# sigp/consensus-specs

Measured on AMD Instinct MI355X. Metric: BLS sig verifications/sec (whole node), higher is better.
Workload: dtype u32 (381-bit Montgomery, 14x28-bit limbs in u32 words); 1 GPU; C2: 65536 independent bls_verify deposit PoP checks per GPU (domain=3, 1/16 tampered); global_batch=65536, parallelism=dp1 (independent items, no collective), batches_in_flight=1, subgroup_policy=pyecc

## Files before the change

consensus-specs_amd/csrc/bls381_field.hpp:

```cpp
#pragma once
#include "bls381_defs.hpp"
#include "bls381_consts.hpp"

namespace bls381 {

#if defined(BLS_COUNT_OPS) && !defined(__HIP_DEVICE_COMPILE__)
inline thread_local uint64_t g_fp_macs = 0;
#define BLS_COUNT_MACS(k) (g_fp_macs += (k))
#else
#define BLS_COUNT_MACS(k) ((void)0)
#endif
#if !defined(__HIP_DEVICE_COMPILE__) && !defined(__HIP__)
inline uint64_t g_inv_fallbacks = 0;
#define BLS_COUNT_INV_FALLBACK() (++g_inv_fallbacks)
#else
#define BLS_COUNT_INV_FALLBACK() ((void)0)
#endif

BLS_INLINE fp_t fp_zero() { fp_t r; for (int i = 0; i < 14; ++i) r.w[i] = 0; return r; }
BLS_INLINE fp_t fp_one() { return FP_ONE_M; }

BLS_INLINE void fp_carry(int32_t (&t)[14]) {
#pragma unroll
  for (int i = 0; i < 13; ++i) {
    t[i + 1] += t[i] >> 28;
    t[i] &= (int32_t)FP_MASK;
  }
}

template <int KMAX>
BLS_INLINE fp_t fp_reduce_lc(const uint32_t (&s)[14]) {
  static_assert(KMAX >= 1 && KMAX <= 8, "value bound");
  int32_t t[14];
  if (KMAX <= 2) {
    const uint32_t m = (int32_t)s[13] > (int32_t)Q2_LIMBS[13] ? ~0u : 0u;
#pragma unroll
    for (int i = 0; i < 14; ++i) t[i] = (int32_t)(s[i] - (Q2_LIMBS[i] & m));
  } else {
    const int32_t top = (int32_t)s[13] > 0 ? (int32_t)s[13] : 0;
    const uint32_t k = (uint32_t)(((uint64_t)(uint32_t)top * LC_DIV_MAGIC) >> 40);
#pragma unroll
    for (int i = 0; i < 14; ++i) t[i] = (int32_t)(s[i] + k * NQ2_LIMBS[i]);
  }
  fp_carry(t);
  if (BLS_ANY(t[13] >= (int32_t)Q2_LIMBS[13])) {
    int32_t e[14];
#pragma unroll
    for (int i = 0; i < 14; ++i) e[i] = t[i] - (int32_t)Q2_LIMBS[i];
    fp_carry(e);
    const bool ge = e[13] >= 0;
#pragma unroll
    for (int i = 0; i < 14; ++i) t[i] = ge ? e[i] : t[i];
  }
  fp_t r;
#pragma unroll
  for (int i = 0; i < 14; ++i) r.w[i] = (uint32_t)t[i];
  return r;
}

BLS_INLINE fp_t fp_add(const fp_t& a, const fp_t& b) {
  uint32_t s[14];
#pragma unroll
  for (int i = 0; i < 14; ++i) s[i] = a.w[i] + b.w[i];
  return fp_reduce_lc<2>(s);
}

BLS_INLINE fp_t fp_sub(const fp_t& a, const fp_t& b) {
  uint32_t s[14];
#pragma unroll
  for (int i = 0; i < 14; ++i) s[i] = a.w[i] + Q2B_LIMBS[i] - b.w[i];
  return fp_reduce_lc<2>(s);
}

BLS_INLINE fp_t fp_neg(const fp_t& a) {
  uint32_t s[14];
#pragma unroll
  for (int i = 0; i < 14; ++i) s[i] = Q2B_LIMBS[i] - a.w[i];
  return fp_reduce_lc<2>(s);
}

BLS_INLINE fp_t fp_dbl(const fp_t& a) {
  uint32_t s[14];
#pragma unroll
  for (int i = 0; i < 14; ++i) s[i] = a.w[i] << 1;
  return fp_reduce_lc<2>(s);
}

BLS_INLINE fp_t fp_add_sub(const fp_t& a, const fp_t& b, const fp_t& c) {
  uint32_t s[14];
#pragma unroll
  for (int i = 0; i < 14; ++i) s[i] = a.w[i] + b.w[i] + Q2B_LIMBS[i] - c.w[i];
  return fp_reduce_lc<3>(s);
}

BLS_INLINE fp_t fp_add3(const fp_t& a, const fp_t& b, const fp_t& c) {
  uint32_t s[14];
#pragma unroll
  for (int i = 0; i < 14; ++i) s[i] = a.w[i] + b.w[i] + c.w[i];
  return fp_reduce_lc<3>(s);
}

BLS_INLINE fp_t fp_sub2(const fp_t& a, const fp_t& b, const fp_t& c) {
  uint32_t s[14];
#pragma unroll
  for (int i = 0; i < 14; ++i) s[i] = a.w[i] + Q4B_LIMBS[i] - b.w[i] - c.w[i];
  return fp_reduce_lc<3>(s);
}

BLS_INLINE fp_t fp_3m2(const fp_t& X, const fp_t& x) {
  uint32_t s[14];
#pragma unroll
  for (int i = 0; i < 14; ++i) s[i] = 3u * X.w[i] + Q4B_LIMBS[i] - (x.w[i] << 1);
  return fp_reduce_lc<5>(s);
}
BLS_INLINE fp_t fp_3p2(const fp_t& X, const fp_t& x) {
  uint32_t s[14];
#pragma unroll
  for (int i = 0; i < 14; ++i) s[i] = 3u * X.w[i] + (x.w[i] << 1);
  return fp_reduce_lc<5>(s);
}
BLS_INLINE fp_t fp_3pm2(const fp_t& X, const fp_t& x, bool minus) {
  uint32_t s[14];
#pragma unroll
  for (int i = 0; i < 14; ++i) {
    const uint32_t x2 = x.w[i] << 1;
    s[i] = 3u * X.w[i] + (minus ? Q4B_LIMBS[i] - x2 : x2);
  }
  return fp_reduce_lc<5>(s);
}

template <int NS> BLS_INLINE uint32_t lc_offset(int i) {
  static_assert(NS >= 2 && NS <= 4, "offsets for two to four subtracted values");
  return NS == 2 ? Q4B_LIMBS[i] : NS == 3 ? Q8T_LIMBS[i] : Q10F_LIMBS[i];
}
constexpr int lc_kmax(int na, int ns) { return na + (ns <= 2 ? ns : ns + 1); }

template <int NA, int NS>
BLS_INLINE fp_t fp_lc(const fp_t* const (&add)[NA], const fp_t* const (&sub)[NS]) {
  static_assert(NA + NS <= 7 && lc_kmax(NA, NS) <= 8, "fp_reduce_lc's limb and value bounds");
  uint32_t s[14];
#pragma unroll
  for (int i = 0; i < 14; ++i) {
    uint32_t v = lc_offset<NS>(i);
#pragma unroll
    for (int j = 0; j < NA; ++j) v += add[j]->w[i];
#pragma unroll
    for (int j = 0; j < NS; ++j) v -= sub[j]->w[i];
    s[i] = v;
  }
  return fp_reduce_lc<lc_kmax(NA, NS)>(s);
}

BLS_INLINE fp_t fp_add_lazy(const fp_t& a, const fp_t& b) {
  fp_t r;
#pragma unroll
  for (int i = 0; i < 14; ++i) r.w[i] = a.w[i] + b.w[i];
  return r;
}

BLS_INLINE fp_t fp_reduce_once(const fp_t& s) {
  int32_t b[14];
#pragma unroll
  for (int i = 0; i < 14; ++i) b[i] = (int32_t)s.w[i] - (int32_t)Q_LIMBS[i];
  fp_carry(b);
  const bool neg = b[13] < 0;
  fp_t r;
#pragma unroll
  for (int i = 0; i < 14; ++i) r.w[i] = neg ? s.w[i] : (uint32_t)b[i];
  return r;
}

BLS_INLINE bool fp_is_zero(const fp_t& a) {
  uint32_t z = 0, e = 0;
#pragma unroll
  for (int i = 0; i < 14; ++i) { z |= a.w[i]; e |= a.w[i] ^ Q_LIMBS[i]; }
  return z == 0 || e == 0;
}

BLS_INLINE bool fp_eq(const fp_t& a, const fp_t& b) { return fp_is_zero(fp_sub(a, b)); }

BLS_INLINE fp_t fp_half(const fp_t& a) {
  const uint32_t odd = a.w[0] & 1u;
  int32_t s[14];
#pragma unroll
  for (int i = 0; i < 14; ++i) s[i] = (int32_t)(a.w[i] + (odd ? Q_LIMBS[i] : 0u));
  fp_carry(s);
  fp_t r;
#pragma unroll
  for (int i = 0; i < 13; ++i) r.w[i] = ((uint32_t)s[i] >> 1) | (((uint32_t)s[i + 1] & 1u) << 27);
  r.w[13] = (uint32_t)s[13] >> 1;
  return r;
}

BLS_INLINE uint64_t fp_mac(uint64_t acc, uint32_t x, uint32_t y) { return BLS_KEEP_ORDER(acc + (uint64_t)x * y); }

template <class F>
BLS_INLINE fp_t fp_mont_columns(const F& col) {
  uint32_t m[14];
  fp_t r;
  uint64_t c = 0;
#pragma unroll
  for (int k = 0; k < 27; ++k) {
    uint64_t acc = col(k, c);
#pragma unroll
    for (int i = (k > 13 ? k - 13 : 0); i < k && i < 14; ++i) acc = fp_mac(acc, m[i], Q_LIMBS[k - i]);
    if (k < 14) {
      m[k] = ((uint32_t)acc * Q_INV28) & FP_MASK;
      acc = fp_mac(acc, m[k], Q_LIMBS[0]);
    } else {
      r.w[k - 14] = (uint32_t)acc & FP_MASK;
    }
    c = acc >> 28;
  }
  r.w[13] = (uint32_t)c & FP_MASK;
  return r;
}

BLS_INLINE fp_t fp_mul_body(const fp_t& a, const fp_t& b) {
  return fp_mont_columns([&](int k, uint64_t acc) {
#pragma unroll
    for (int i = (k > 13 ? k - 13 : 0); i <= k && i < 14; ++i) acc = fp_mac(acc, a.w[i], b.w[k - i]);
    return acc;
  });
}

BLS_INLINE fp_t fp_sqr_body(const fp_t& a) {
  uint32_t a2[14];
#pragma unroll
  for (int i = 0; i < 14; ++i) a2[i] = a.w[i] << 1;
  return fp_mont_columns([&](int k, uint64_t acc) {
#pragma unroll
    for (int i = (k > 13 ? k - 13 : 0); 2 * i < k; ++i) acc = fp_mac(acc, a2[i], a.w[k - i]);
    if ((k & 1) == 0) acc = fp_mac(acc, a.w[k / 2], a.w[k / 2]);
    return acc;
  });
}

#if defined(__clang__)
typedef uint32_t fpv_t __attribute__((ext_vector_type(14)));
BLS_INLINE fpv_t fp_pack(const fp_t& a) {
  fpv_t v;
#pragma unroll
  for (int k = 0; k < 14; ++k) v[k] = a.w[k];
  return v;
}
BLS_INLINE fp_t fp_unpack(const fpv_t& v) {
  fp_t a;
#pragma unroll
  for (int k = 0; k < 14; ++k) a.w[k] = v[k];
  return a;
}
BLS_NOINLINE fpv_t fp_mul_call(fpv_t a, fpv_t b) { return fp_pack(fp_mul_body(fp_unpack(a), fp_unpack(b))); }
BLS_NOINLINE fpv_t fp_sqr_call(fpv_t a) { return fp_pack(fp_sqr_body(fp_unpack(a))); }
BLS_INLINE fp_t fp_mul(const fp_t& a, const fp_t& b) { return fp_unpack(fp_mul_call(fp_pack(a), fp_pack(b))); }
BLS_INLINE fp_t fp_sqr(const fp_t& a) { return fp_unpack(fp_sqr_call(fp_pack(a))); }
#else
BLS_NOINLINE fp_t fp_mul(fp_t a, fp_t b) { BLS_COUNT_MACS(392); return fp_mul_body(a, b); }
BLS_NOINLINE fp_t fp_sqr(fp_t a) { BLS_COUNT_MACS(301); return fp_sqr_body(a); }
#endif

BLS_INLINE fp_t fp_mul_small(const fp_t& a, int k) {
  if (k <= 8) {
    uint32_t s[14];
#pragma unroll
    for (int i = 0; i < 14; ++i) s[i] = (uint32_t)k * a.w[i];
    return fp_reduce_lc<8>(s);
  }
  fp_t r = a;
  fp_t acc = fp_zero();
  bool first = true;
  while (k) {
    if (k & 1) { acc = first ? r : fp_add(acc, r); first = false; }
    k >>= 1;
    if (k) r = fp_dbl(r);
  }
  return acc;
}

BLS_DEV_INLINE fp_t fp_pow_limbs(const fp_t& a, const uint32_t* e, int nbits) {
  fp_t r = FP_ONE_M;
  for (int i = nbits - 1; i >= 0; --i) {
    r = fp_sqr(r);
    if ((e[i >> 5] >> (i & 31)) & 1u) r = fp_mul(r, a);
  }
  return r;
}

BLS_HD inline fp_t fp_pow_qm3d4(const fp_t a) {
  const fp_t a2 = fp_sqr(a);
  const fp_t t1 = a, t3 = fp_mul(t1, a2), t5 = fp_mul(t3, a2), t7 = fp_mul(t5, a2);
  const fp_t t9 = fp_mul(t7, a2), t11 = fp_mul(t9, a2), t13 = fp_mul(t11, a2), t15 = fp_mul(t13, a2);
  fp_t r = FP_ONE_M;
  for (int k = 0; k < POW_QM3D4_NSTEPS; ++k) {
    for (int j = POW_QM3D4_SQR[k]; j > 0; --j) r = fp_sqr(r);
    switch (POW_QM3D4_DIG[k]) {
      case 1: r = fp_mul(r, t1); break;
      case 3: r = fp_mul(r, t3); break;
      case 5: r = fp_mul(r, t5); break;
      case 7: r = fp_mul(r, t7); break;
      case 9: r = fp_mul(r, t9); break;
      case 11: r = fp_mul(r, t11); break;
      case 13: r = fp_mul(r, t13); break;
      case 15: r = fp_mul(r, t15); break;
      default: break;
    }
  }
  return r;
}

BLS_HD inline fp_t fp_inv(const fp_t am);

BLS_DEV_INLINE bool fp_sqrt(fp_t& r, const fp_t& a) {
  r = fp_mul(fp_pow_qm3d4(a), a);
  return fp_eq(fp_sqr(r), a);
}

BLS_INLINE fp_t fp_to_mont(const fp_t& plain) { return fp_mul(plain, FP_R2); }
BLS_INLINE fp_t fp_from_mont(const fp_t& m) {
  fp_t one = fp_zero();
  one.w[0] = 1;
  return fp_reduce_once(fp_mul(m, one));
}

BLS_INLINE bool fp_plain_lt_q(const fp_t& a) {
  int32_t b[14];
#pragma unroll
  for (int i = 0; i < 14; ++i) b[i] = (int32_t)a.w[i] - (int32_t)Q_LIMBS[i];
  fp_carry(b);
  return b[13] < 0;
}

BLS_INLINE bool fp_plain_is_zero(const fp_t& a) {
  uint32_t z = 0;
#pragma unroll
  for (int i = 0; i < 14; ++i) z |= a.w[i];
  return z == 0;
}

BLS_INLINE bool fp_plain_gt(const fp_t& a, const fp_t& b) {
  int32_t d[14];
#pragma unroll
  for (int i = 0; i < 14; ++i) d[i] = (int32_t)b.w[i] - (int32_t)a.w[i];
  fp_carry(d);
// ... 748 lines not shown
```

consensus-specs_amd/csrc/bls381_lazy.hpp:

```cpp
#pragma once
#include "bls381_field.hpp"

namespace bls381 {

struct wide_t { int64_t c[28]; };
typedef int32_t lv_t[14];

constexpr int WIDE_OFF_SHIFT = 22;

BLS_INLINE void wz_init(wide_t& T) {
#pragma unroll
  for (int k = 0; k < 28; ++k) T.c[k] = 0;
#pragma unroll
  for (int j = 0; j < 14; ++j) T.c[13 + j] = (int64_t)Q_LIMBS[j] << WIDE_OFF_SHIFT;
}

BLS_INLINE void wmac(wide_t& T, const lv_t& x, const lv_t& y) {
  BLS_COUNT_MACS(196);
#pragma unroll
  for (int i = 0; i < 14; ++i)
#pragma unroll
    for (int j = 0; j < 14; ++j) T.c[i + j] += (int64_t)x[i] * (int64_t)y[j];
}

BLS_INLINE void wmac_init(wide_t& T, const lv_t& x, const lv_t& y) {
  BLS_COUNT_MACS(196);
#pragma unroll
  for (int i = 0; i < 14; ++i)
#pragma unroll
    for (int j = 0; j < 14; ++j) {
      const int k = i + j;
      const int64_t p = (int64_t)x[i] * (int64_t)y[j];
      if (i == 0 || j == 13)
        T.c[k] = p + ((k >= 13) ? ((int64_t)Q_LIMBS[k - 13] << WIDE_OFF_SHIFT) : 0);
      else
        T.c[k] += p;
    }
  T.c[27] = 0;
}

BLS_INLINE void wsqr_k(wide_t& T, const lv_t& x, int32_t k) {
  BLS_COUNT_MACS(105);
#pragma unroll
  for (int i = 0; i < 14; ++i) {
    const int32_t d = k * x[i], c = 2 * k * x[i];
    T.c[2 * i] += (int64_t)d * (int64_t)x[i];
#pragma unroll
    for (int j = i + 1; j < 14; ++j) T.c[i + j] += (int64_t)c * (int64_t)x[j];
  }
}

BLS_INLINE fp_t wredc(wide_t& T) {
  BLS_COUNT_MACS(196);
#pragma unroll
  for (int i = 0; i < 14; ++i) {
    const uint32_t m = ((uint32_t)T.c[i] * Q_INV28) & FP_MASK;
#pragma unroll
    for (int j = 0; j < 14; ++j) T.c[i + j] = (int64_t)((uint64_t)T.c[i + j] + (uint64_t)m * Q_LIMBS[j]);
    T.c[i + 1] += T.c[i] >> 28;
  }
  fp_t r;
  int64_t c = 0;
#pragma unroll
  for (int j = 0; j < 14; ++j) {
    const int64_t v = T.c[14 + j] + c;
    r.w[j] = (uint32_t)v & FP_MASK;
    c = v >> 28;
  }
  return r;
}

BLS_INLINE void lv_from(lv_t& r, const fp_t& a) {
#pragma unroll
  for (int k = 0; k < 14; ++k) r[k] = (int32_t)a.w[k];
}

BLS_INLINE fp_t fp_6p2(const fp_t& X, const fp_t& x) {
  uint32_t s[14];
#pragma unroll
  for (int i = 0; i < 14; ++i) s[i] = 6u * X.w[i] + (x.w[i] << 1);
  return fp_reduce_lc<6>(s);
}

BLS_INLINE fp_t fp_6p2_3m2(bool six, const fp_t& P, const fp_t& S, const fp_t& x) {
  uint32_t s[14];
#pragma unroll
  for (int i = 0; i < 14; ++i) {
    const uint32_t x2 = x.w[i] << 1;
    s[i] = six ? 6u * P.w[i] + x2 : 3u * S.w[i] + Q4B_LIMBS[i] - x2;
  }
  return fp_reduce_lc<6>(s);
}


BLS_INLINE fp_t lz_xi_mul(bool p, const fp_t& a0, const fp_t& a1, const fp_t& b0, const fp_t& b1) {
  lv_t x1, y1, x2, y2;
#pragma unroll
  for (int k = 0; k < 14; ++k) {
    const int32_t s = (int32_t)b0.w[k] + (int32_t)b1.w[k];
    const int32_t d = (int32_t)b0.w[k] - (int32_t)b1.w[k];
    x1[k] = (int32_t)a0.w[k];
    x2[k] = (int32_t)a1.w[k];
    y1[k] = p ? s : d;
    y2[k] = p ? d : -s;
  }
  wide_t T;
  wmac_init(T, x1, y1);
  wmac(T, x2, y2);
  return wredc(T);
}

BLS_INLINE fp_t lz_mul(bool p, const fp_t& a0, const fp_t& a1, const fp_t& b0, const fp_t& b1) {
  lv_t x1, y1, x2, y2;
#pragma unroll
  for (int k = 0; k < 14; ++k) {
    x1[k] = (int32_t)a0.w[k];
    x2[k] = (int32_t)a1.w[k];
    y1[k] = (int32_t)(p ? b1.w[k] : b0.w[k]);
    y2[k] = p ? (int32_t)b0.w[k] : -(int32_t)b1.w[k];
  }
  wide_t T;
  wmac_init(T, x1, y1);
  wmac(T, x2, y2);
  return wredc(T);
}

BLS_INLINE fp_t lz_sqr_xisqr(bool p, const fp_t& a0, const fp_t& a1, const fp_t& b0, const fp_t& b1) {
  lv_t x1, y1, u, v;
#pragma unroll
  for (int k = 0; k < 14; ++k) {
    const int32_t e = (int32_t)a0.w[k], o = (int32_t)a1.w[k];
    x1[k] = e + (p ? e : o);
    y1[k] = p ? o : e - o;
    const int32_t c = (int32_t)b0.w[k], d = (int32_t)b1.w[k];
    u[k] = p ? c + d : c - d;
    v[k] = d;
  }
  wide_t T;
  wmac_init(T, x1, y1);
  wsqr_k(T, u, 1);
  wsqr_k(T, v, -2);
  return wredc(T);
}

}
```

consensus-specs_amd/csrc/dev_check.hip:

```cpp
#include <cstring>
#include <vector>

#include "bls381_quad.hpp"

using namespace bls381;

namespace {

#define DC_OPS(X)                      \
  X(P_MUL, 2, 2, 2, 1, 0)              \
  X(P_SQR, 2, 2, 1, 1, 0)              \
  X(P_CONJ, 2, 2, 1, 1, 0)             \
  X(P_MUL_XI, 2, 2, 1, 1, 0)           \
  X(P_ADD_MUL_XI, 2, 2, 2, 1, 0)       \
  X(P_SUB2, 2, 2, 3, 1, 0)             \
  X(P_3PM2, 2, 2, 2, 1, 0)             \
  X(P_MUL_SMALL, 2, 2, 1, 1, 0)        \
  X(P_INV, 2, 2, 1, 1, 0)              \
  X(P_PRED, 2, 2, 2, 1, 0)             \
  X(P12_MUL, 2, 2, 12, 6, 0)           \
  X(P12_SQR, 2, 2, 6, 6, 0)            \
  X(P12_CYC_SQR, 2, 2, 6, 6, 0)        \
  X(P12_MUL_BY_LINE, 2, 2, 9, 6, 0)    \
  X(P12_FROB, 2, 2, 6, 18, 0)          \
  X(P12_INV, 2, 2, 6, 6, 0)            \
  X(P_CSQR, 2, 2, 4, 4, 0)             \
  X(P12_FINAL_EXP, 2, 2, 6, 6, 1)      \
  X(P12_FINAL_EXP_NOFB, 2, 2, 6, 6, 1) \
  X(Q_MUL, 4, 4, 6, 3, 0)              \
  X(Q_SQR, 4, 4, 3, 3, 0)              \
  X(Q_TWO_LINES, 4, 4, 3, 3, 0)        \
  X(Q_MUL_BY_LINE, 4, 4, 6, 3, 0)      \
  X(Q_FROB, 4, 4, 3, 9, 0)             \
  X(Q_INV, 4, 4, 3, 3, 0)              \
  X(Q_CONJ, 4, 4, 3, 3, 0)             \
  X(Q_CSQR, 4, 4, 3, 2, 1)             \
  X(Q_DECOMPRESS, 4, 4, 3, 3, 0)       \
  X(Q_CYC_EXP_X, 4, 4, 3, 6, 1)        \
  X(Q_FINAL_EXP, 4, 4, 3, 3, 1)        \
  X(O_MUL, 8, 4, 6, 3, 0)              \
  X(O_SQR, 8, 4, 3, 3, 0)              \
  X(O_MUL_BY_LINE, 8, 4, 6, 3, 0)      \
  X(O_CSQR, 8, 4, 3, 2, 1)             \
  X(O_CYC_EXP_X, 8, 4, 3, 9, 1)        \
  X(O_FINAL_EXP_OQ, 8, 4, 3, 3, 1)     \
  X(O_FINAL_EXP_OO, 8, 4, 3, 3, 1)     \
  X(G_DBL_Q, 4, 4, 3, 3, 1)            \
  X(G_ADD_AFF_Q, 4, 4, 5, 3, 1)        \
  X(G_ADD_Q, 4, 4, 6, 3, 1)            \
  X(G_PSI_Q, 4, 4, 3, 3, 1)            \
  X(G_MUL_U64_Q, 4, 4, 2, 3, 1)        \
  X(G_MUL_BP_Q, 4, 4, 2, 3, 1)         \
  X(G_DBL_O, 8, 4, 3, 3, 1)            \
  X(G_MUL_U64_O, 8, 4, 2, 3, 1)        \
  X(G_MUL_BP_O, 8, 4, 2, 3, 1)         \
  X(M_QUAD, 4, 4, 4, 3, 1)             \
  X(M_Q1, 4, 4, 4, 3, 1)               \
  X(M_O1, 8, 4, 4, 3, 1)               \
  X(P_ADD_XI_SUB2, 2, 2, 4, 1, 0)      \
  X(P_SUB2_ADD_XI, 2, 2, 4, 1, 0)      \
  X(P_SUB2_ADD, 2, 2, 4, 1, 0)         \
  X(P_SUB_SUB_XI, 2, 2, 3, 1, 0)       \
  X(P_SUB_SUB_DBL, 2, 2, 3, 1, 0)      \
  X(P_DBL_SUB2, 2, 2, 3, 1, 0)         \
  X(P_3A_XI_B_M2C, 2, 2, 3, 1, 0)      \
  X(P_2A_B_M3C, 2, 2, 3, 1, 0)

enum dc_op : int {
#define X(name, g, gin, nin, nout, pad) name,
  DC_OPS(X)
#undef X
      DC_NOPS
};
struct op_info { const char* name; int g, gin, nin, nout, pad; };
constexpr op_info OPS[DC_NOPS] = {
#define X(name, g, gin, nin, nout, pad) {#name, g, gin, nin, nout, pad},
    DC_OPS(X)
#undef X
};

typedef __attribute__((address_space(1))) const uint32_t g_cu32;
typedef __attribute__((address_space(1))) uint32_t g_u32;
typedef __attribute__((address_space(1))) const uint64_t g_cu64;

__device__ __forceinline__ fp_t lane_ld(const uint32_t* __restrict__ p, size_t L, size_t lane, int slot) {
  g_cu32* g = (g_cu32*)p;
  fp_t r;
#pragma unroll
  for (int k = 0; k < FP_LIMBS; ++k) r.w[k] = g[(size_t)(slot * FP_LIMBS + k) * L + lane];
  return r;
}
__device__ __forceinline__ void lane_st(uint32_t* __restrict__ p, size_t L, size_t lane, int slot, const fp_t& a) {
  g_u32* g = (g_u32*)p;
#pragma unroll
  for (int k = 0; k < FP_LIMBS; ++k) g[(size_t)(slot * FP_LIMBS + k) * L + lane] = a.w[k];
}

using fp12p_t = fp12_g<fp2p_t>;
__device__ __forceinline__ fp12p_t mk12(const fp_t* I) {
  fp12p_t f;
  f.c0.c0 = pr_make(I[0]); f.c0.c1 = pr_make(I[1]); f.c0.c2 = pr_make(I[2]);
  f.c1.c0 = pr_make(I[3]); f.c1.c1 = pr_make(I[4]); f.c1.c2 = pr_make(I[5]);
  return f;
}
__device__ __forceinline__ void put12(fp_t* O, const fp12p_t& f) {
  O[0] = f.c0.c0.v; O[1] = f.c0.c1.v; O[2] = f.c0.c2.v; O[3] = f.c1.c0.v; O[4] = f.c1.c1.v; O[5] = f.c1.c2.v;
}
__device__ __forceinline__ fq12_t mkq(const fp_t* I) {
  fq12_t f;
  f.h.c0 = pr_make(I[0]); f.h.c1 = pr_make(I[1]); f.h.c2 = pr_make(I[2]);
  return f;
}
__device__ __forceinline__ void putq(fp_t* O, const fq12_t& f) { O[0] = f.h.c0.v; O[1] = f.h.c1.v; O[2] = f.h.c2.v; }
__device__ __forceinline__ jac_t<fp2p_t> mkjac(const fp_t* I) {
  jac_t<fp2p_t> p; p.x = pr_make(I[0]); p.y = pr_make(I[1]); p.z = pr_make(I[2]); return p;
}
__device__ __forceinline__ aff_t<fp2p_t> mkaff(const fp_t* I) {
  aff_t<fp2p_t> p; p.x = pr_make(I[0]); p.y = pr_make(I[1]); return p;
}
__device__ __forceinline__ void putjac(fp_t* O, uint32_t& fl, const jac_t<fp2p_t>& p) {
  O[0] = p.x.v; O[1] = p.y.v; O[2] = p.z.v;
  fl = jac_is_inf(p) ? 1u : 0u;
}
__device__ __forceinline__ g1_line_pre mkg1(const fp_t* I) {
  aff_t<fp_t> P; P.x = I[0]; P.y = I[1];
  return g1_prepare(P);
}
__device__ __forceinline__ bool snapshot_g2_zero(const fq12_t& f) {
  cq_t g = cq_compress(f);
  bool zero = false;
  for (int s = 0; s < 6; ++s) {
    for (int j = CYC_X_RUNS_RTL[s]; j > 0; --j) g = cq_sqr(g);
    zero = zero | fp2_is_zero(cq_g2(g));
  }
  return zero;
}

template <int OP>
__device__ __forceinline__ void probe(const fp_t* I, uint64_t aux, fp_t* O, uint32_t& fl) {
  if constexpr (OP == P_MUL) O[0] = fp2_mul(pr_make(I[0]), pr_make(I[1])).v;
  else if constexpr (OP == P_SQR) O[0] = fp2_sqr(pr_make(I[0])).v;
  else if constexpr (OP == P_CONJ) O[0] = fp2_conj(pr_make(I[0])).v;
  else if constexpr (OP == P_MUL_XI) O[0] = fp2_mul_xi(pr_make(I[0])).v;
  else if constexpr (OP == P_ADD_MUL_XI) O[0] = fp2_add_mul_xi(pr_make(I[0]), pr_make(I[1])).v;
  else if constexpr (OP == P_SUB2) O[0] = fp2_sub2(pr_make(I[0]), pr_make(I[1]), pr_make(I[2])).v;
  else if constexpr (OP == P_3PM2) O[0] = fp2_3pm2(pr_make(I[0]), pr_make(I[1]), aux != 0).v;
  else if constexpr (OP == P_MUL_SMALL) O[0] = fp2_mul_small(pr_make(I[0]), (int)aux).v;
  else if constexpr (OP == P_INV) O[0] = fp2_inv(pr_make(I[0])).v;
  else if constexpr (OP == P_PRED) {
    const fp2p_t a = pr_make(I[0]), b = pr_make(I[1]);
    const fp_t a0 = pr_dpp<DPP_EVEN>(a.v), b0 = pr_dpp<DPP_EVEN>(b.v);
    fl = (fp2_is_zero(a) ? 1u : 0u) | (fp2_eq(a, b) ? 2u : 0u) | (pr_both(fp_eq(a0, b0)) ? 4u : 0u);
    O[0] = fp_zero();
  } else if constexpr (OP == P12_MUL) put12(O, fp12_mul(mk12(I), mk12(I + 6)));
  else if constexpr (OP == P12_SQR) put12(O, fp12_sqr(mk12(I)));
  else if constexpr (OP == P12_CYC_SQR) put12(O, fp12_cyclotomic_sqr(mk12(I)));
  else if constexpr (OP == P12_MUL_BY_LINE)
    put12(O, fp12_mul_by_line(mk12(I), pr_make(I[6]), pr_make(I[7]), pr_make(I[8])));
  else if constexpr (OP == P12_FROB) {
    for (int p = 1; p <= 3; ++p) put12(O + 6 * (p - 1), fp12_frob(mk12(I), p));
  } else if constexpr (OP == P12_INV) put12(O, fp12_inv(mk12(I)));
  else if constexpr (OP == P_CSQR) {
    cyc_bc<fp2p_t> g;
    g.g2 = pr_make(I[0]); g.g3 = pr_make(I[1]); g.g4 = pr_make(I[2]); g.g5 = pr_make(I[3]);
    for (uint64_t j = 0; j < aux; ++j) g = cyc_csqr(g);
    O[0] = g.g2.v; O[1] = g.g3.v; O[2] = g.g4.v; O[3] = g.g5.v;
  } else if constexpr (OP == P12_FINAL_EXP) put12(O, final_exp(mk12(I)));
  else if constexpr (OP == P12_FINAL_EXP_NOFB) {
    const fe_ct<fp2p_t> r = final_exp_ct<fp2p_t, 0>(mk12(I));
    const bool z0 = fp2_is_zero(r.c.c0.c0), z1 = fp2_is_zero(r.c.c1.c0);
    const bool one = fp12_eq(r.c, fp12_conj(r.t3));
    fl = (z0 && z1) ? 2u : (one ? 1u : 0u);
    put12(O, fp12_mul_inl(r.c, r.t3));
  } else if constexpr (OP == Q_MUL) putq(O, fq12_mul(mkq(I), mkq(I + 3)));
  else if constexpr (OP == Q_SQR) putq(O, fq12_sqr(mkq(I)));
  else if constexpr (OP == Q_TWO_LINES) putq(O, fq12_two_lines(pr_make(I[0]), pr_make(I[1]), pr_make(I[2])));
  else if constexpr (OP == Q_MUL_BY_LINE)
    putq(O, fq12_mul_by_line_q1(mkq(I), pr_make(I[3]), pr_make(I[4]), pr_make(I[5])));
  else if constexpr (OP == Q_FROB) {
    for (int p = 1; p <= 3; ++p) putq(O + 3 * (p - 1), fq12_frob(mkq(I), p));
  } else if constexpr (OP == Q_INV) putq(O, fq12_inv(mkq(I)));
  else if constexpr (OP == Q_CONJ) {
    putq(O, fq12_conj(mkq(I)));
    fl = fq12_is_one(mkq(I)) ? 1u : 0u;
  } else if constexpr (OP == Q_CSQR) {
    cq_t g = cq_compress(mkq(I));
    bool zero = false;
    for (uint64_t j = 0; j < aux; ++j) {
      g = cq_sqr(g);
      zero = zero | fp2_is_zero(cq_g2(g));
    }
    O[0] = g.x.v; O[1] = g.y.v;
    fl = zero ? 1u : 0u;
  } else if constexpr (OP == Q_DECOMPRESS) {
    cq_t g;
    g.x = pr_make(I[0]); g.y = pr_make(I[1]);
    putq(O, cq_decompress(g, pr_make(I[2])));
  } else if constexpr (OP == Q_CYC_EXP_X) {
    putq(O, cyc_exp_x_lg<on_quad, csqr_on_quad>(mkq(I)));
    putq(O + 3, cyc_exp_x_gs_lg<on_quad>(mkq(I)));
    fl = snapshot_g2_zero(mkq(I)) ? 1u : 0u;
  } else if constexpr (OP == Q_FINAL_EXP) putq(O, final_exp_lg<on_quad, csqr_on_quad>(mkq(I)));
  else if constexpr (OP == O_MUL) putq(O, fq12_mul_oct(mkq(I), mkq(I + 3)));
  else if constexpr (OP == O_SQR) putq(O, fq12_sqr_oct(mkq(I)));
  else if constexpr (OP == O_MUL_BY_LINE)
    putq(O, fq12_mul_by_line_oct(mkq(I), pr_make(I[3]), pr_make(I[4]), pr_make(I[5])));
  else if constexpr (OP == O_CSQR) {
    fp2p_t g = co_enter(cq_compress(mkq(I)));
    for (uint64_t j = 0; j < aux; ++j) g = co_sqr(g);
    const cq_t r = co_exit(g);
    O[0] = r.x.v; O[1] = r.y.v;
    fl = fp2_is_zero(cq_g2(r)) ? 1u : 0u;
  } else if constexpr (OP == O_CYC_EXP_X) {
    putq(O, cyc_exp_x_lg<on_octet, csqr_on_quad>(mkq(I)));
    putq(O + 3, cyc_exp_x_lg<on_octet, csqr_on_octet>(mkq(I)));
    putq(O + 6, cyc_exp_x_gs_lg<on_octet>(mkq(I)));
    fl = snapshot_g2_zero(mkq(I)) ? 1u : 0u;
  } else if constexpr (OP == O_FINAL_EXP_OQ) putq(O, final_exp_lg<on_octet, csqr_on_quad>(mkq(I)));
  else if constexpr (OP == O_FINAL_EXP_OO) putq(O, final_exp_lg<on_octet, csqr_on_octet>(mkq(I)));
  else if constexpr (OP == G_DBL_Q) putjac(O, fl, jac_dbl_q(mkjac(I)));
  else if constexpr (OP == G_ADD_AFF_Q) putjac(O, fl, jac_add_aff_q(mkjac(I), mkaff(I + 3)));
  else if constexpr (OP == G_ADD_Q) putjac(O, fl, jac_add_q(mkjac(I), mkjac(I + 3)));
  else if constexpr (OP == G_PSI_Q) putjac(O, fl, g2_psi_jac_q(mkjac(I)));
  else if constexpr (OP == G_MUL_U64_Q) putjac(O, fl, jac_mul_u64_lg<on_quad>(mkaff(I), aux));
  else if constexpr (OP == G_MUL_BP_Q) putjac(O, fl, g2_mul_bp_lg<on_quad>(mkaff(I)));
  else if constexpr (OP == G_DBL_O) putjac(O, fl, jac_dbl_o(mkjac(I)));
  else if constexpr (OP == G_MUL_U64_O) putjac(O, fl, jac_mul_u64_lg<on_octet>(mkaff(I), aux));
  else if constexpr (OP == G_MUL_BP_O) putjac(O, fl, g2_mul_bp_lg<on_octet>(mkaff(I)));
  else if constexpr (OP == M_QUAD) {
    const bool active = ((aux >> (qd_hi() ? 1 : 0)) & 1u) != 0;
    bool degen = false;
    putq(O, miller_loop_quad(mkaff(I), mkg1(I + 2), active, degen));
    fl = degen ? 1u : 0u;
  } else if constexpr (OP == M_Q1) {
    bool degen = false;
    putq(O, miller_loop_lg<on_quad>(mkaff(I), mkg1(I + 2), degen));
    fl = degen ? 1u : 0u;
  } else if constexpr (OP == M_O1) {
    const fq12_ml r = miller_loop_lg_run<on_octet>(mkaff(I), mkg1(I + 2));
    putq(O, r.f);
    fl = r.degenerate ? 1u : 0u;
  } else if constexpr (OP == P_ADD_XI_SUB2)
    O[0] = fp2_add_xi_sub2(pr_make(I[0]), pr_make(I[1]), pr_make(I[2]), pr_make(I[3])).v;
  else if constexpr (OP == P_SUB2_ADD_XI)
    O[0] = fp2_sub2_add_xi(pr_make(I[0]), pr_make(I[1]), pr_make(I[2]), pr_make(I[3])).v;
  else if constexpr (OP == P_SUB2_ADD)
    O[0] = fp2_sub2_add(pr_make(I[0]), pr_make(I[1]), pr_make(I[2]), pr_make(I[3])).v;
  else if constexpr (OP == P_SUB_SUB_XI) O[0] = fp2_sub_sub_xi(pr_make(I[0]), pr_make(I[1]), pr_make(I[2])).v;
  else if constexpr (OP == P_SUB_SUB_DBL) O[0] = fp2_sub_sub_dbl(pr_make(I[0]), pr_make(I[1]), pr_make(I[2])).v;
  else if constexpr (OP == P_DBL_SUB2) O[0] = fp2_dbl_sub2(pr_make(I[0]), pr_make(I[1]), pr_make(I[2])).v;
  else if constexpr (OP == P_3A_XI_B_M2C) O[0] = fp2_3a_xi_b_m2c(pr_make(I[0]), pr_make(I[1]), pr_make(I[2])).v;
  else if constexpr (OP == P_2A_B_M3C) O[0] = fp2_2a_b_m3c(pr_make(I[0]), pr_make(I[1]), pr_make(I[2])).v;
}

template <int OP>
__global__ void __launch_bounds__(64) k_probe(const uint32_t* __restrict__ in, const uint64_t* __restrict__ aux,
                                              uint32_t* __restrict__ out, uint32_t* __restrict__ flag, size_t L,
                                              size_t live) {
  constexpr int NIN = OPS[OP].nin, NOUT = OPS[OP].nout;
  const size_t lane = (size_t)blockIdx.x * 64 + threadIdx.x;
  fp_t I[NIN], O[NOUT];
#pragma unroll
  for (int j = 0; j < NIN; ++j) I[j] = lane_ld(in, L, lane, j);
  const uint64_t ax = ((g_cu64*)aux)[lane];
  uint32_t fl = 0;
  probe<OP>(I, ax, O, fl);
  if (lane >= live) return;
#pragma unroll
  for (int j = 0; j < NOUT; ++j) lane_st(out, L, lane, j, O[j]);
  ((g_u32*)flag)[lane] = fl;
}

template <int OP>
hipError_t launch(int op, size_t L, size_t live, const uint32_t* in, const uint64_t* aux, uint32_t* out,
                  uint32_t* flag) {
  if constexpr (OP < DC_NOPS) {
    if (op != OP) return launch<OP + 1>(op, L, live, in, aux, out, flag);
    hipLaunchKernelGGL(k_probe<OP>, dim3((unsigned)(L / 64)), dim3(64), 0, 0, in, aux, out, flag, L, live);
    return hipGetLastError();
  } else {
    return hipErrorInvalidValue;
  }
}

}

extern "C" {

int dc_op_count() { return DC_NOPS; }
const char* dc_op_name(int op) { return (op >= 0 && op < DC_NOPS) ? OPS[op].name : nullptr; }
int dc_op_info(int op, int info[4]) {
  if (op < 0 || op >= DC_NOPS) return -1;
  info[0] = OPS[op].g; info[1] = OPS[op].gin; info[2] = OPS[op].nin; info[3] = OPS[op].nout;
  return 0;
}

int dc_run(int op, size_t n, const uint32_t* in, const uint64_t* aux, uint32_t* out, uint32_t* flag) {
  if (op < 0 || op >= DC_NOPS || n == 0 || n > 4096) return (int)hipErrorInvalidValue;
  const op_info& o = OPS[op];
  const size_t per_wave = 64 / (size_t)o.g;
  const size_t n_pad = (n + per_wave - 1) / per_wave * per_wave;
  const size_t L = n_pad * o.g, live = n * o.g;
  std::vector<uint32_t> hin((size_t)o.nin * FP_LIMBS * L, 0u), hout((size_t)o.nout * FP_LIMBS * L);
  std::vector<uint64_t> haux(L, 0u);
  std::vector<uint32_t> hflag(L);
  for (size_t i = 0; i < n_pad; ++i) {
    if (i >= n && !o.pad) continue;
    const size_t src = i < n ? i : 0;
    for (int l = 0; l < o.g; ++l) {
      const size_t lane = i * o.g + l;
      haux[lane] = aux ? aux[src] : 0;
      for (int j = 0; j < o.nin; ++j)
        for (int k = 0; k < FP_LIMBS; ++k)
          hin[(size_t)(j * FP_LIMBS + k) * L + lane] = in[((src * o.nin + j) * o.gin + (size_t)(l % o.gin)) * FP_LIMBS + k];
    }
  }
  uint32_t *din = nullptr, *dout = nullptr, *dflag = nullptr;
  uint64_t* daux = nullptr;
  hipError_t e = hipMalloc(&din, hin.size() * 4);
  if (e == hipSuccess) e = hipMalloc(&dout, hout.size() * 4);
  if (e == hipSuccess) e = hipMalloc(&dflag, L * 4);
  if (e == hipSuccess) e = hipMalloc(&daux, L * 8);
  if (e == hipSuccess) e = hipMemcpy(din, hin.data(), hin.size() * 4, hipMemcpyHostToDevice);
  if (e == hipSuccess) e = hipMemcpy(daux, haux.data(), L * 8, hipMemcpyHostToDevice);
  if (e == hipSuccess) e = launch<0>(op, L, live, din, daux, dout, dflag);
  if (e == hipSuccess) e = hipDeviceSynchronize();
  if (e == hipSuccess) e = hipMemcpy(hout.data(), dout, hout.size() * 4, hipMemcpyDeviceToHost);
  if (e == hipSuccess) e = hipMemcpy(hflag.data(), dflag, L * 4, hipMemcpyDeviceToHost);
  (void)hipFree(din); (void)hipFree(dout); (void)hipFree(dflag); (void)hipFree(daux);
  if (e != hipSuccess) return (int)e;
  for (size_t i = 0; i < n; ++i)
    for (int l = 0; l < o.g; ++l) {
      const size_t lane = i * o.g + l;
      flag[lane] = hflag[lane];
      for (int j = 0; j < o.nout; ++j)
        for (int k = 0; k < FP_LIMBS; ++k)
          out[((i * o.nout + j) * o.g + l) * FP_LIMBS + k] = hout[(size_t)(j * FP_LIMBS + k) * L + lane];
    }
  return 0;
}

}
```

Before: 2.550 million verifications/s.

## Fuse lazy Fp2 products into column-wise Montgomery reduction to cut register pressure

After: 2.583 million verifications/s, median of 6. 1.01x the previous value.

```diff
diff --git a/consensus-specs_amd/csrc/bls381_field.hpp b/consensus-specs_amd/csrc/bls381_field.hpp
--- a/consensus-specs_amd/csrc/bls381_field.hpp
+++ b/consensus-specs_amd/csrc/bls381_field.hpp
@@ -28,17 +28,25 @@
   }
 }
 
+BLS_INLINE uint32_t fp_opaque(uint32_t x) {
+#if defined(__HIP_DEVICE_COMPILE__)
+  asm("" : "+v"(x));
+#endif
+  return x;
+}
+BLS_INLINE uint32_t fp_lane_mask(bool c) { return fp_opaque(c ? ~0u : 0u); }
+
 template <int KMAX>
 BLS_INLINE fp_t fp_reduce_lc(const uint32_t (&s)[14]) {
   static_assert(KMAX >= 1 && KMAX <= 8, "value bound");
   int32_t t[14];
   if (KMAX <= 2) {
-    const uint32_t m = (int32_t)s[13] > (int32_t)Q2_LIMBS[13] ? ~0u : 0u;
-#pragma unroll
-    for (int i = 0; i < 14; ++i) t[i] = (int32_t)(s[i] - (Q2_LIMBS[i] & m));
+    const uint32_t m = fp_lane_mask((int32_t)s[13] > (int32_t)Q2_LIMBS[13]);
+#pragma unroll
+    for (int i = 0; i < 14; ++i) t[i] = (int32_t)(s[i] + (NQ2_LIMBS[i] & m));
   } else {
-    const int32_t top = (int32_t)s[13] > 0 ? (int32_t)s[13] : 0;
-    const uint32_t k = (uint32_t)(((uint64_t)(uint32_t)top * LC_DIV_MAGIC) >> 40);
+    const uint32_t top = fp_opaque((uint32_t)((int32_t)s[13] > 0 ? s[13] : 0u));
+    const uint32_t k = (uint32_t)(((uint64_t)top * LC_DIV_MAGIC) >> 40);
 #pragma unroll
     for (int i = 0; i < 14; ++i) t[i] = (int32_t)(s[i] + k * NQ2_LIMBS[i]);
   }
diff --git a/consensus-specs_amd/csrc/bls381_lazy.hpp b/consensus-specs_amd/csrc/bls381_lazy.hpp
--- a/consensus-specs_amd/csrc/bls381_lazy.hpp
+++ b/consensus-specs_amd/csrc/bls381_lazy.hpp
@@ -21,22 +21,6 @@
   for (int i = 0; i < 14; ++i)
 #pragma unroll
     for (int j = 0; j < 14; ++j) T.c[i + j] += (int64_t)x[i] * (int64_t)y[j];
-}
-
-BLS_INLINE void wmac_init(wide_t& T, const lv_t& x, const lv_t& y) {
-  BLS_COUNT_MACS(196);
-#pragma unroll
-  for (int i = 0; i < 14; ++i)
-#pragma unroll
-    for (int j = 0; j < 14; ++j) {
-      const int k = i + j;
-      const int64_t p = (int64_t)x[i] * (int64_t)y[j];
-      if (i == 0 || j == 13)
-        T.c[k] = p + ((k >= 13) ? ((int64_t)Q_LIMBS[k - 13] << WIDE_OFF_SHIFT) : 0);
-      else
-        T.c[k] += p;
-    }
-  T.c[27] = 0;
 }
 
 BLS_INLINE void wsqr_k(wide_t& T, const lv_t& x, int32_t k) {
@@ -68,6 +52,43 @@
     c = v >> 28;
   }
   return r;
+}
+
+BLS_INLINE int64_t wz_mac(int64_t acc, int32_t x, int32_t y) { return BLS_KEEP_ORDER(acc + (int64_t)x * (int64_t)y); }
+
+template <class F>
+BLS_INLINE fp_t wredc_columns(const F& col) {
+  int32_t m[14];
+  fp_t r;
+  int64_t c = 0;
+#pragma unroll
+  for (int k = 0; k < 27; ++k) {
+    int64_t acc = col(k, c);
+#pragma unroll
+    for (int i = (k > 13 ? k - 13 : 0); i < k && i < 14; ++i) acc = wz_mac(acc, m[i], (int32_t)Q_LIMBS[k - i]);
+    if (k < 14) {
+      const uint32_t lo = (uint32_t)acc + (k == 13 ? Q_LIMBS[0] << WIDE_OFF_SHIFT : 0u);
+      m[k] = (int32_t)(((lo * Q_INV28) & FP_MASK) + (k == 13 ? 1u << WIDE_OFF_SHIFT : 0u));
+      acc = wz_mac(acc, m[k], (int32_t)Q_LIMBS[0]);
+    } else {
+      r.w[k - 14] = (uint32_t)acc & FP_MASK;
+    }
+    c = acc >> 28;
+  }
+  r.w[13] = (uint32_t)c & FP_MASK;
+  return r;
+}
+
+BLS_INLINE int64_t wcol_mul(int k, int64_t acc, const lv_t& x, const lv_t& y) {
+#pragma unroll
+  for (int i = (k > 13 ? k - 13 : 0); i <= k && i < 14; ++i) acc = wz_mac(acc, x[i], y[k - i]);
+  return acc;
+}
+BLS_INLINE int64_t wcol_sqr(int k, int64_t acc, const lv_t& x, const lv_t& d, const lv_t& c) {
+#pragma unroll
+  for (int i = (k > 13 ? k - 13 : 0); 2 * i < k; ++i) acc = wz_mac(acc, c[i], x[k - i]);
+  if ((k & 1) == 0) acc = wz_mac(acc, d[k / 2], x[k / 2]);
+  return acc;
 }
 
 BLS_INLINE void lv_from(lv_t& r, const fp_t& a) {
@@ -104,10 +125,8 @@
     y1[k] = p ? s : d;
     y2[k] = p ? d : -s;
   }
-  wide_t T;
-  wmac_init(T, x1, y1);
-  wmac(T, x2, y2);
-  return wredc(T);
+  BLS_COUNT_MACS(588);
+  return wredc_columns([&](int k, int64_t acc) { return wcol_mul(k, wcol_mul(k, acc, x1, y1), x2, y2); });
 }
 
 BLS_INLINE fp_t lz_mul(bool p, const fp_t& a0, const fp_t& a1, const fp_t& b0, const fp_t& b1) {
@@ -119,14 +138,12 @@
     y1[k] = (int32_t)(p ? b1.w[k] : b0.w[k]);
     y2[k] = p ? (int32_t)b0.w[k] : -(int32_t)b1.w[k];
   }
-  wide_t T;
-  wmac_init(T, x1, y1);
-  wmac(T, x2, y2);
-  return wredc(T);
+  BLS_COUNT_MACS(588);
+  return wredc_columns([&](int k, int64_t acc) { return wcol_mul(k, wcol_mul(k, acc, x1, y1), x2, y2); });
 }
 
 BLS_INLINE fp_t lz_sqr_xisqr(bool p, const fp_t& a0, const fp_t& a1, const fp_t& b0, const fp_t& b1) {
-  lv_t x1, y1, u, v;
+  lv_t x1, y1, u, u2, v, vm2, vm4;
 #pragma unroll
   for (int k = 0; k < 14; ++k) {
     const int32_t e = (int32_t)a0.w[k], o = (int32_t)a1.w[k];
@@ -134,13 +151,15 @@
     y1[k] = p ? o : e - o;
     const int32_t c = (int32_t)b0.w[k], d = (int32_t)b1.w[k];
     u[k] = p ? c + d : c - d;
+    u2[k] = 2 * u[k];
     v[k] = d;
+    vm2[k] = -2 * d;
+    vm4[k] = -4 * d;
   }
-  wide_t T;
-  wmac_init(T, x1, y1);
-  wsqr_k(T, u, 1);
-  wsqr_k(T, v, -2);
-  return wredc(T);
+  BLS_COUNT_MACS(602);
+  return wredc_columns([&](int k, int64_t acc) {
+    return wcol_sqr(k, wcol_sqr(k, wcol_mul(k, acc, x1, y1), u, u, u2), v, vm2, vm4);
+  });
 }
 
 }
diff --git a/consensus-specs_amd/csrc/dev_check.hip b/consensus-specs_amd/csrc/dev_check.hip
--- a/consensus-specs_amd/csrc/dev_check.hip
+++ b/consensus-specs_amd/csrc/dev_check.hip
@@ -64,7 +64,10 @@
   X(P_SUB_SUB_DBL, 2, 2, 3, 1, 0)      \
   X(P_DBL_SUB2, 2, 2, 3, 1, 0)         \
   X(P_3A_XI_B_M2C, 2, 2, 3, 1, 0)      \
-  X(P_2A_B_M3C, 2, 2, 3, 1, 0)
+  X(P_2A_B_M3C, 2, 2, 3, 1, 0)        \
+  X(P_ADD, 2, 2, 2, 1, 0)              \
+  X(P_SUB, 2, 2, 2, 1, 0)              \
+  X(P_DBL, 2, 2, 1, 1, 0)
 
 enum dc_op : int {
 #define X(name, g, gin, nin, nout, pad) name,
@@ -251,14 +254,17 @@
   else if constexpr (OP == P_DBL_SUB2) O[0] = fp2_dbl_sub2(pr_make(I[0]), pr_make(I[1]), pr_make(I[2])).v;
   else if constexpr (OP == P_3A_XI_B_M2C) O[0] = fp2_3a_xi_b_m2c(pr_make(I[0]), pr_make(I[1]), pr_make(I[2])).v;
   else if constexpr (OP == P_2A_B_M3C) O[0] = fp2_2a_b_m3c(pr_make(I[0]), pr_make(I[1]), pr_make(I[2])).v;
-}
-
-template <int OP>
-__global__ void __launch_bounds__(64) k_probe(const uint32_t* __restrict__ in, const uint64_t* __restrict__ aux,
+  else if constexpr (OP == P_ADD) O[0] = fp2_add(pr_make(I[0]), pr_make(I[1])).v;
+  else if constexpr (OP == P_SUB) O[0] = fp2_sub(pr_make(I[0]), pr_make(I[1])).v;
+  else if constexpr (OP == P_DBL) O[0] = fp2_dbl(pr_make(I[0])).v;
+}
+
+template <int OP, int BLOCK>
+__global__ void __launch_bounds__(BLOCK) k_probe(const uint32_t* __restrict__ in, const uint64_t* __restrict__ aux,
                                               uint32_t* __restrict__ out, uint32_t* __restrict__ flag, size_t L,
                                               size_t live) {
   constexpr int NIN = OPS[OP].nin, NOUT = OPS[OP].nout;
-  const size_t lane = (size_t)blockIdx.x * 64 + threadIdx.x;
+  const size_t lane = (size_t)blockIdx.x * BLOCK + threadIdx.x;
   fp_t I[NIN], O[NOUT];
 #pragma unroll
   for (int j = 0; j < NIN; ++j) I[j] = lane_ld(in, L, lane, j);
@@ -271,12 +277,24 @@
   ((g_u32*)flag)[lane] = fl;
 }
 
+constexpr bool wg_probe(int op) { return OPS[op].g == 2 && OPS[op].nin <= 4 && OPS[op].nout <= 4; }
+
 template <int OP>
 hipError_t launch(int op, size_t L, size_t live, const uint32_t* in, const uint64_t* aux, uint32_t* out,
-                  uint32_t* flag) {
+                  uint32_t* flag, int block) {
   if constexpr (OP < DC_NOPS) {
-    if (op != OP) return launch<OP + 1>(op, L, live, in, aux, out, flag);
-    hipLaunchKernelGGL(k_probe<OP>, dim3((unsigned)(L / 64)), dim3(64), 0, 0, in, aux, out, flag, L, live);
+    if (op != OP) return launch<OP + 1>(op, L, live, in, aux, out, flag, block);
+    if (block == 64) {
+      hipLaunchKernelGGL((k_probe<OP, 64>), dim3((unsigned)(L / 64)), dim3(64), 0, 0, in, aux, out, flag, L, live);
+    } else {
+      if constexpr (wg_probe(OP)) {
+        if (block != KBLOCK || L % KBLOCK) return hipErrorInvalidValue;
+        hipLaunchKernelGGL((k_probe<OP, KBLOCK>), dim3((unsigned)(L / KBLOCK)), dim3(KBLOCK), 0, 0, in, aux, out, flag,
+                           L, live);
+      } else {
+        return hipErrorInvalidValue;
+      }
+    }
     return hipGetLastError();
   } else {
     return hipErrorInvalidValue;
@@ -295,10 +313,12 @@
   return 0;
 }
 
-int dc_run(int op, size_t n, const uint32_t* in, const uint64_t* aux, uint32_t* out, uint32_t* flag) {
+}
+namespace {
+int run(int op, size_t n, const uint32_t* in, const uint64_t* aux, uint32_t* out, uint32_t* flag, int block) {
   if (op < 0 || op >= DC_NOPS || n == 0 || n > 4096) return (int)hipErrorInvalidValue;
   const op_info& o = OPS[op];
-  const size_t per_wave = 64 / (size_t)o.g;
+  const size_t per_wave = (size_t)block / (size_t)o.g;
   const size_t n_pad = (n + per_wave - 1) / per_wave * per_wave;
   const size_t L = n_pad * o.g, live = n * o.g;
   std::vector<uint32_t> hin((size_t)o.nin * FP_LIMBS * L, 0u), hout((size_t)o.nout * FP_LIMBS * L);
@@ -323,7 +343,7 @@
   if (e == hipSuccess) e = hipMalloc(&daux, L * 8);
   if (e == hipSuccess) e = hipMemcpy(din, hin.data(), hin.size() * 4, hipMemcpyHostToDevice);
   if (e == hipSuccess) e = hipMemcpy(daux, haux.data(), L * 8, hipMemcpyHostToDevice);
-  if (e == hipSuccess) e = launch<0>(op, L, live, din, daux, dout, dflag);
+  if (e == hipSuccess) e = launch<0>(op, L, live, din, daux, dout, dflag, block);
   if (e == hipSuccess) e = hipDeviceSynchronize();
   if (e == hipSuccess) e = hipMemcpy(hout.data(), dout, hout.size() * 4, hipMemcpyDeviceToHost);
   if (e == hipSuccess) e = hipMemcpy(hflag.data(), dflag, L * 4, hipMemcpyDeviceToHost);
@@ -339,5 +359,14 @@
     }
   return 0;
 }
-
-}
+}
+extern "C" {
+
+int dc_run(int op, size_t n, const uint32_t* in, const uint64_t* aux, uint32_t* out, uint32_t* flag) {
+  return run(op, n, in, aux, out, flag, 64);
+}
+int dc_run_wg(int op, size_t n, const uint32_t* in, const uint64_t* aux, uint32_t* out, uint32_t* flag) {
+  return run(op, n, in, aux, out, flag, KBLOCK);
+}
+
+}
```
